# DCDmllm/AnyEdit

Measured on NVIDIA H100. Metric: edited images/sec (512x512, 50-step DDIM, CFG), higher is better.
Workload: dtype f16

## Files before the change

### anyedit_b200/_lib.py

```python
import ctypes as C
import os

_HERE = os.path.dirname(os.path.abspath(__file__))
LIB_PATH = os.path.join(_HERE, "libanysd_b200.so")

F32, F16, I64 = 0, 1, 2
EINVAL, ECUDA, EUNSUPPORTED = -1, -2, -3


class GemmParams(C.Structure):
    _fields_ = [
        ("A", C.c_void_p), ("W", C.c_void_p), ("bias", C.c_void_p), ("rowadd", C.c_void_p),
        ("residual", C.c_void_p), ("out", C.c_void_p),
        ("M", C.c_int), ("N", C.c_int), ("K", C.c_int),
        ("lda", C.c_int), ("ldw", C.c_int), ("ldo", C.c_int), ("ldr", C.c_int), ("ld_rowadd", C.c_int),
        ("rows_per_batch", C.c_int), ("act", C.c_int), ("out_dtype", C.c_int), ("conv", C.c_int),
        ("Nimg", C.c_int), ("H", C.c_int), ("Wd", C.c_int), ("Cin", C.c_int),
        ("stride", C.c_int), ("upsample", C.c_int),
        ("workspace", C.c_void_p), ("workspace_bytes", C.c_size_t),
        ("conv_pad", C.c_int),
        ("stats", C.c_void_p), ("stats_images", C.c_int),
        ("splitk_workspace", C.c_void_p), ("splitk_workspace_bytes", C.c_size_t),
        ("splitk_counters", C.c_void_p), ("splitk_counters_bytes", C.c_size_t),
        ("row_stats", C.c_void_p), ("ln_stats", C.c_void_p), ("ln_colsum", C.c_void_p), ("ln_eps", C.c_float),
# ... 48 lines not shown
    "anysd_add_nchw_into_nhwc_f16": (_I, [_VP, _I, _VP, _I, _I, _I, _I, _VP]),
    "anysd_nhwc_to_nchw": (_I, [_VP, _I, _I, _VP, _I, _I, _I, _I, _I, _VP]),
    "anysd_concat_channels_f16": (_I, [_VP, _I, _VP, _I, _VP, _LL, _VP]),
    "anysd_cast_f32_to_f16": (_I, [_VP, _VP, _LL, _VP]),
    "anysd_timestep_embedding_f16": (_I, [_VP, _I, _VP, _I, _I, _F, _VP]),
    "anysd_emb_finalize": (_I, [_VP, _VP, _VP, _I, _VP, _VP, _I, _I, _VP]),
    "anysd_router_gate_f32": (_I, [_VP, _VP, _I, _VP, _VP, _VP, _I, _I, _I, _I, _VP]),
    "anysd_groupnorm_workspace_bytes": (_SZ, [_I, _I, _I]),
    "anysd_groupnorm_resident": (_I, [_I, _I, _I, _I]),
    "anysd_groupnorm_nhwc_f16": (_I, [_VP, _I, _VP, _I, _VP, _VP, _VP, _I, _I, _I, _F, _I, _VP, _SZ, _VP]),
    "anysd_layernorm_f16": (_I, [_VP, _VP, _VP, _VP, _LL, _I, _F, _VP]),
    "anysd_gemm_f16": (_I, [C.POINTER(GemmParams), _VP]),
    "anysd_gemm_stats_slabs": (_I, [C.POINTER(GemmParams)]),
    "anysd_gemm_splitk_workspace_bytes": (_SZ, [C.POINTER(GemmParams)]),
    "anysd_geglu_ff_f16": (_I, [_VP, _I, _VP, _VP, _VP, _VP, _VP, _I, _VP, _I, _I, _I, _I, _VP]),
    "anysd_groupnorm_apply_nhwc_f16": (_I, [_VP, _I, _VP, _I, _VP, _I, _VP, _VP, _VP, _I, _I, _I, _F, _I, _VP, _SZ, _VP]),
    "anysd_attention_f16": (_I, [C.POINTER(AttnParams), _VP]),
    "anysd_cfg_ddim_step_f32": (_I, [_VP, _VP, _VP, _VP, _F, _I, _I, _VP, _VP, _LL, _I, _VP]),
    "anysd_cfg3_ddim_step_f32": (_I, [_VP, _VP, _VP, _VP, _F, _F, _VP, _VP, _LL, _I, _VP]),
    "anysd_cfg_plms_step_f32": (_I, [_VP, _VP, _VP, _F, _I, _VP, _VP, _VP, _LL, _I, _VP]),
    "anysd_cfg_dpmpp_step_f32": (_I, [_VP, _VP, _VP, _F, _I, _VP, _VP, _VP, _LL, _I, _VP]),
    "anysd_softmax_rows_f32": (_I, [_VP, _LL, _VP, _LL, _I, _I, _F, _VP]),
    "anysd_gaussian_posterior_f32": (_I, [_VP, _VP, _VP, _VP, _F, _I, _LL, _VP]),
    "anysd_embed_tokens_f16": (_I, [_VP, _VP, _VP, _VP, _I, _I, _I, _I, _VP]),
    "anysd_attention_small_f16": (_I, [_VP, _VP, _VP, _VP, _I, _I, _I, _I, _I, _I, _I, _I, _I, _F, _I, _VP]),
    "anysd_resize_bilinear_f16": (_I, [_VP, _VP, _VP, _I, _I, _I, _I, _I, _I, _I, _I, _VP]),
    "anysd_resize_bilinear_ac_f32": (_I, [_VP, _VP, _I, _I, _I, _I, _I, _VP]),
    "anysd_relu_f16": (_I, [_VP, _VP, _LL, _VP]),
    "anysd_depth_to_space_f16": (_I, [_VP, _VP, _I, _I, _I, _I, _I, _VP]),
    "anysd_space_to_depth_f16": (_I, [_VP, _VP, _I, _I, _I, _I, _I, _VP]),
# ... 67 lines not shown
```

### anyedit_b200/csrc/common.cuh

```cuda
#pragma once
#include <cuda_fp16.h>
#include <cuda_runtime.h>
#include <stdint.h>
#include <stdio.h>

#include "../../include/anysd_b200.h"

namespace anysd {

void set_error(const char* fmt, ...);
int check_launch(const char* what);

#define ANYSD_REQUIRE(cond, code, ...)                 \
    do {                                               \
        if (!(cond)) {                                 \
            ::anysd::set_error(__VA_ARGS__);           \
            return (code);                             \
        }                                              \
    } while (0)

static inline int cdiv(long long a, long long b) { return (int)((a + b - 1) / b); }

int sm_count();

// ... 35 lines not shown
#pragma unroll
    for (int i = 0; i < 4; ++i) {
        float2 t = __half22float2(h[i]);
        f[2 * i] = t.x;
        f[2 * i + 1] = t.y;
    }
}
__device__ __forceinline__ uint4 pack8(const float* f) {
    uint4 u;
    __half2* h = reinterpret_cast<__half2*>(&u);
#pragma unroll
    for (int i = 0; i < 4; ++i) h[i] = __floats2half2_rn(f[2 * i], f[2 * i + 1]);
    return u;
}

__device__ __forceinline__ uint32_t smem_u32(const void* p) {
    return (uint32_t)__cvta_generic_to_shared(p);
}

__device__ __forceinline__ void cp_async16(uint32_t dst, const void* src, bool valid) {
    int sz = valid ? 16 : 0;
    asm volatile("cp.async.cg.shared.global [%0], [%1], 16, %2;\n" ::"r"(dst), "l"(src), "r"(sz));
}
__device__ __forceinline__ void cp_async_commit() { asm volatile("cp.async.commit_group;\n" ::); }
template <int N>
__device__ __forceinline__ void cp_async_wait() {
    asm volatile("cp.async.wait_group %0;\n" ::"n"(N));
}

__device__ __forceinline__ void ldmatrix_x4(uint32_t& r0, uint32_t& r1, uint32_t& r2, uint32_t& r3, uint32_t addr) {
// ... 18 lines not shown
```

### anyedit_b200/csrc/norm.cu

```cuda
#include "common.cuh"

namespace anysd {

constexpr int GN_MAX_SPLITS = 64;
constexpr int GN_U = 8;

__device__ __forceinline__ float silu_fast(float v) {
    float e, r;
    asm("ex2.approx.ftz.f32 %0, %1;" : "=f"(e) : "f"(v * -1.4426950408889634f));
    asm("rcp.approx.ftz.f32 %0, %1;" : "=f"(r) : "f"(1.0f + e));
    return v * r;
}

struct GnGeom {
    int CV;
    int CV1;
    int R;
    int T;
};

static GnGeom gn_geom(int C1, int C2) {
    GnGeom g;
    g.CV = (C1 + C2) / 8;
    g.CV1 = C1 / 8;
// ... 471 lines not shown
template <int LPR, int VPL>
__global__ void layernorm_kernel(const uint4* __restrict__ x, const float* __restrict__ gamma,
                                 const float* __restrict__ beta, uint4* __restrict__ y, long long M, int CV, float eps) {
    constexpr int RPW = 32 / LPR;
    const int lane = threadIdx.x & 31;
    const int sub = lane / LPR, l = lane % LPR;
    const long long row = ((long long)blockIdx.x * (blockDim.x >> 5) + (threadIdx.x >> 5)) * RPW + sub;
    const bool row_ok = row < M;
    const uint4* xr = x + (row_ok ? row : 0) * CV;
    float f[VPL][8];
    float s = 0.f;
#pragma unroll
    for (int i = 0; i < VPL; ++i) {
        const int v = l + i * LPR;
        if (v < CV) {
            uint4 u = __ldg(xr + v);
            unpack8(u, f[i]);
#pragma unroll
            for (int j = 0; j < 8; ++j) s += f[i][j];
        }
    }
#pragma unroll
    for (int o = LPR / 2; o > 0; o >>= 1) s += __shfl_xor_sync(0xffffffffu, s, o);
    const float inv_c = 1.0f / (float)(CV * 8);
    const float mean = s * inv_c;
    float q = 0.f;
#pragma unroll
    for (int i = 0; i < VPL; ++i) {
        const int v = l + i * LPR;
        if (v < CV) {
#pragma unroll
            for (int j = 0; j < 8; ++j) {
                float d = f[i][j] - mean;
                q += d * d;
            }
        }
    }
#pragma unroll
    for (int o = LPR / 2; o > 0; o >>= 1) q += __shfl_xor_sync(0xffffffffu, q, o);
    const float rstd = rsqrtf(q * inv_c + eps);
    if (!row_ok) return;
    uint4* yr = y + row * CV;
#pragma unroll
    for (int i = 0; i < VPL; ++i) {
        const int v = l + i * LPR;
        if (v < CV) {
            const float4* g4 = reinterpret_cast<const float4*>(gamma + v * 8);
            const float4* b4 = reinterpret_cast<const float4*>(beta + v * 8);
            float4 g0 = __ldg(g4), g1 = __ldg(g4 + 1), b0 = __ldg(b4), b1 = __ldg(b4 + 1);
            float gg[8] = {g0.x, g0.y, g0.z, g0.w, g1.x, g1.y, g1.z, g1.w};
            float bb[8] = {b0.x, b0.y, b0.z, b0.w, b1.x, b1.y, b1.z, b1.w};
            float o[8];
#pragma unroll
            for (int j = 0; j < 8; ++j) o[j] = (f[i][j] - mean) * rstd * gg[j] + bb[j];
            yr[v] = pack8(o);
        }
    }
}

}

using namespace anysd;

extern "C" {

int anysd_groupnorm_resident(int C1, int C2, int HW, int G) {
    GnResPlan pl;
    return gn_res_plan(C1, C2 < 0 ? 0 : C2, HW, G, &pl) ? 1 : 0;
}

size_t anysd_groupnorm_workspace_bytes(int N, int G, int C) {
// ... 125 lines not shown
```

### anyedit_b200/csrc/wgmma.cuh

```cuda
#pragma once
#include <stdint.h>

namespace anysd {

__device__ __forceinline__ void wg_fence() { asm volatile("wgmma.fence.sync.aligned;" ::: "memory"); }
__device__ __forceinline__ void wg_commit() { asm volatile("wgmma.commit_group.sync.aligned;" ::: "memory"); }
template <int N>
__device__ __forceinline__ void wg_wait() { asm volatile("wgmma.wait_group.sync.aligned %0;" ::"n"(N) : "memory"); }
__device__ __forceinline__ void wg_fence_regs(float& r) { asm volatile("" : "+f"(r)::"memory"); }

__device__ __forceinline__ uint64_t wg_desc(uint32_t addr, uint32_t lbo_bytes, uint32_t sbo_bytes) {
    return (uint64_t)((addr >> 4) & 0x3FFF) | ((uint64_t)((lbo_bytes >> 4) & 0x3FFF) << 16) |
           ((uint64_t)((sbo_bytes >> 4) & 0x3FFF) << 32) | (1ull << 62);
}

template <int N>
struct Wgmma;

template <>
struct Wgmma<16> {
    static __device__ __forceinline__ void ss(float* d, uint64_t a, uint64_t b, int scale_d) {
        asm volatile(
            "{\n\t.reg .pred p;\n\tsetp.ne.b32 p, %10, 0;\n\t"
            "wgmma.mma_async.sync.aligned.m64n16k16.f32.f16.f16 {%0, %1, %2, %3, %4, %5, %6, %7}, %8, %9, p, 1, 1, 0, 0;\n\t}"
// ... 56 lines not shown
            "{\n\t.reg .pred p;\n\tsetp.ne.b32 p, %37, 0;\n\t"
            "wgmma.mma_async.sync.aligned.m64n64k16.f32.f16.f16 {%0, %1, %2, %3, %4, %5, %6, %7, %8, %9, %10, %11, %12, %13, %14, %15, %16, %17, %18, %19, %20, %21, %22, %23, %24, %25, %26, %27, %28, %29, %30, %31}, {%32, %33, %34, %35}, %36, p, 1, 1, 1;\n\t}"
            : "+f"(d[0]), "+f"(d[1]), "+f"(d[2]), "+f"(d[3]), "+f"(d[4]), "+f"(d[5]), "+f"(d[6]), "+f"(d[7]), "+f"(d[8]), "+f"(d[9]), "+f"(d[10]), "+f"(d[11]), "+f"(d[12]), "+f"(d[13]), "+f"(d[14]), "+f"(d[15]), "+f"(d[16]), "+f"(d[17]), "+f"(d[18]), "+f"(d[19]), "+f"(d[20]), "+f"(d[21]), "+f"(d[22]), "+f"(d[23]), "+f"(d[24]), "+f"(d[25]), "+f"(d[26]), "+f"(d[27]), "+f"(d[28]), "+f"(d[29]), "+f"(d[30]), "+f"(d[31])
            : "r"(a[0]), "r"(a[1]), "r"(a[2]), "r"(a[3]), "l"(b), "r"(scale_d));
    }
};
template <>
struct Wgmma<80> {
    static __device__ __forceinline__ void ss(float* d, uint64_t a, uint64_t b, int scale_d) {
        asm volatile(
            "{\n\t.reg .pred p;\n\tsetp.ne.b32 p, %42, 0;\n\t"
            "wgmma.mma_async.sync.aligned.m64n80k16.f32.f16.f16 {%0, %1, %2, %3, %4, %5, %6, %7, %8, %9, %10, %11, %12, %13, %14, %15, %16, %17, %18, %19, %20, %21, %22, %23, %24, %25, %26, %27, %28, %29, %30, %31, %32, %33, %34, %35, %36, %37, %38, %39}, %40, %41, p, 1, 1, 0, 0;\n\t}"
            : "+f"(d[0]), "+f"(d[1]), "+f"(d[2]), "+f"(d[3]), "+f"(d[4]), "+f"(d[5]), "+f"(d[6]), "+f"(d[7]), "+f"(d[8]), "+f"(d[9]), "+f"(d[10]), "+f"(d[11]), "+f"(d[12]), "+f"(d[13]), "+f"(d[14]), "+f"(d[15]), "+f"(d[16]), "+f"(d[17]), "+f"(d[18]), "+f"(d[19]), "+f"(d[20]), "+f"(d[21]), "+f"(d[22]), "+f"(d[23]), "+f"(d[24]), "+f"(d[25]), "+f"(d[26]), "+f"(d[27]), "+f"(d[28]), "+f"(d[29]), "+f"(d[30]), "+f"(d[31]), "+f"(d[32]), "+f"(d[33]), "+f"(d[34]), "+f"(d[35]), "+f"(d[36]), "+f"(d[37]), "+f"(d[38]), "+f"(d[39])
            : "l"(a), "l"(b), "r"(scale_d));
    }
    static __device__ __forceinline__ void rs_t(float* d, const uint32_t* a, uint64_t b, int scale_d) {
        asm volatile(
            "{\n\t.reg .pred p;\n\tsetp.ne.b32 p, %45, 0;\n\t"
            "wgmma.mma_async.sync.aligned.m64n80k16.f32.f16.f16 {%0, %1, %2, %3, %4, %5, %6, %7, %8, %9, %10, %11, %12, %13, %14, %15, %16, %17, %18, %19, %20, %21, %22, %23, %24, %25, %26, %27, %28, %29, %30, %31, %32, %33, %34, %35, %36, %37, %38, %39}, {%40, %41, %42, %43}, %44, p, 1, 1, 1;\n\t}"
            : "+f"(d[0]), "+f"(d[1]), "+f"(d[2]), "+f"(d[3]), "+f"(d[4]), "+f"(d[5]), "+f"(d[6]), "+f"(d[7]), "+f"(d[8]), "+f"(d[9]), "+f"(d[10]), "+f"(d[11]), "+f"(d[12]), "+f"(d[13]), "+f"(d[14]), "+f"(d[15]), "+f"(d[16]), "+f"(d[17]), "+f"(d[18]), "+f"(d[19]), "+f"(d[20]), "+f"(d[21]), "+f"(d[22]), "+f"(d[23]), "+f"(d[24]), "+f"(d[25]), "+f"(d[26]), "+f"(d[27]), "+f"(d[28]), "+f"(d[29]), "+f"(d[30]), "+f"(d[31]), "+f"(d[32]), "+f"(d[33]), "+f"(d[34]), "+f"(d[35]), "+f"(d[36]), "+f"(d[37]), "+f"(d[38]), "+f"(d[39])
            : "r"(a[0]), "r"(a[1]), "r"(a[2]), "r"(a[3]), "l"(b), "r"(scale_d));
    }
};
template <>
struct Wgmma<96> {
    static __device__ __forceinline__ void ss(float* d, uint64_t a, uint64_t b, int scale_d) {
        asm volatile(
            "{\n\t.reg .pred p;\n\tsetp.ne.b32 p, %50, 0;\n\t"
            "wgmma.mma_async.sync.aligned.m64n96k16.f32.f16.f16 {%0, %1, %2, %3, %4, %5, %6, %7, %8, %9, %10, %11, %12, %13, %14, %15, %16, %17, %18, %19, %20, %21, %22, %23, %24, %25, %26, %27, %28, %29, %30, %31, %32, %33, %34, %35, %36, %37, %38, %39, %40, %41, %42, %43, %44, %45, %46, %47}, %48, %49, p, 1, 1, 0, 0;\n\t}"
            : "+f"(d[0]), "+f"(d[1]), "+f"(d[2]), "+f"(d[3]), "+f"(d[4]), "+f"(d[5]), "+f"(d[6]), "+f"(d[7]), "+f"(d[8]), "+f"(d[9]), "+f"(d[10]), "+f"(d[11]), "+f"(d[12]), "+f"(d[13]), "+f"(d[14]), "+f"(d[15]), "+f"(d[16]), "+f"(d[17]), "+f"(d[18]), "+f"(d[19]), "+f"(d[20]), "+f"(d[21]), "+f"(d[22]), "+f"(d[23]), "+f"(d[24]), "+f"(d[25]), "+f"(d[26]), "+f"(d[27]), "+f"(d[28]), "+f"(d[29]), "+f"(d[30]), "+f"(d[31]), "+f"(d[32]), "+f"(d[33]), "+f"(d[34]), "+f"(d[35]), "+f"(d[36]), "+f"(d[37]), "+f"(d[38]), "+f"(d[39]), "+f"(d[40]), "+f"(d[41]), "+f"(d[42]), "+f"(d[43]), "+f"(d[44]), "+f"(d[45]), "+f"(d[46]), "+f"(d[47])
// ... 114 lines not shown
```

### anyedit_b200/ops.py

```python
import os
import ctypes as C

import torch

from . import _lib
from ._lib import F16, F32, I64, AttnParams, GemmParams

_DT = {torch.float32: F32, torch.float16: F16, torch.int64: I64}

launch_count = 0


def _stream():
    return C.c_void_p(torch.cuda.current_stream().cuda_stream)


def _ptr(t):
    return C.c_void_p(t.data_ptr()) if t is not None else None


def _cuda(*ts):
    for t in ts:
        if t is not None and not t.is_cuda:
            raise _lib.AnysdError("anysd_b200 ops need CUDA tensors; there is no CPU fallback")
# ... 236 lines not shown
    _cuda(x, w1, b1, w2t, b2, residual, out)
    Cc = x.shape[-1]
    M = x.numel() // Cc
    hidden = w2t.shape[0]
    assert w1.shape == (2 * hidden, Cc) and w2t.shape == (hidden, Cc) and b1.numel() == 2 * hidden
    assert b1.dtype == torch.float32 and b2.dtype == torch.float32 and b1.is_contiguous() and b2.is_contiguous()
    assert w1.is_contiguous() and w2t.is_contiguous()
    fl = 2.0 * M * (2 * hidden) * Cc + 2.0 * M * Cc * hidden
    with _Traced("gemm", fl, f"ff-geglu M={M} C={Cc} hidden={hidden}"):
        _lib.check(_lib.load().anysd_geglu_ff_f16(_ptr(x), x.stride(-2), _ptr(w1), _ptr(b1), _ptr(w2t), _ptr(b2),
                                                  _ptr(residual), residual.stride(-2), _ptr(out), out.stride(-2), M, Cc,
                                                  hidden, _stream()), "geglu_ff")
    _count()


def conv3x3(x, W, out, bias=None, rowadd=None, residual=None, stride=1, upsample=0, ld_rowadd=None,
            logical_cin=None, logical_cout=None, act=0, pad_rb=False, stats=False):
    _cuda(x, W, out)
    Nimg, H, Wd, Cin = x.shape
    Hl, Wl = H << upsample, Wd << upsample
    if pad_rb:
        assert stride == 2 and not upsample
        Ho, Wo = (Hl - 2) // 2 + 1, (Wl - 2) // 2 + 1
    else:
        Ho, Wo = (Hl - 1) // stride + 1, (Wl - 1) // stride + 1
    p = GemmParams()
    p.A, p.W, p.out = x.data_ptr(), W.data_ptr(), out.data_ptr()
    p.bias = bias.data_ptr() if bias is not None else None
    p.rowadd = rowadd.data_ptr() if rowadd is not None else None
    p.residual = residual.data_ptr() if residual is not None else None
# ... 477 lines not shown
```

### anyedit_b200/unet.py

```python
import math
import os

import torch
import torch.nn as nn

from . import ops



class _Param(nn.Module):

    def __init__(self, wshape, bias=True, kind="linear", zero=False):
        super().__init__()
        self.kind = kind
        self.weight = nn.Parameter(torch.empty(*wshape))
        if bias:
            self.bias = nn.Parameter(torch.empty(wshape[0]))
        else:
            self.register_parameter("bias", None)
        self.reset(zero)

    @torch.no_grad()
    def reset(self, zero=False):
        if self.kind == "norm":
# ... 99 lines not shown
        super().__init__()
        self.conv = _Param((out_ch, ch, 3, 3), kind="conv")


class _Embedding(nn.Module):
    def __init__(self, n, d):
        super().__init__()
        self.weight = nn.Parameter(torch.randn(n, d))



_LN_FOLD = os.environ.get("ANYSD_LN_FOLD", "0")[:1] == "1"


FF_FUSED_C = 320


def ff1_chunk_order(hidden, chunk=32):
    idx = []
    for c in range(hidden // chunk):
        for P in range(chunk):
            i, q = divmod(P, 4)
            u = c * chunk + 16 * (i // 4) + (2 * q, 2 * q + 1, 2 * q + 8, 2 * q + 9)[i % 4]
            idx += [2 * u, 2 * u + 1]
    return torch.tensor(idx, dtype=torch.long)


def _h(t, dev):
    return t.detach().to(device=dev, dtype=torch.float16).contiguous()

# ... 452 lines not shown
                ops.gemm(xq, ln[1]["w"], qkv, bias=ln[1]["b"], ln=(ln[0], ln[1]["cs"], 1e-5))
            else:
                ops.gemm(xq, ad["qkv_w"], qkv, bias=ad["qkv_b"])
            ops.attention(qkv, qkv[:, Cp:], qkv[:, 2 * Cp:], a, N, ad["heads"], n_q, n_q, ad["d"],
                          3 * Cp, 3 * Cp, 3 * Cp, C, head_stride=hs, aux_cols=ad["aux"])
        else:
            L = ctx.shape[1]
            if q_pre is not None:
                q = q_pre
            else:
                q = torch.empty(N * n_q, Cp, dtype=torch.float16, device=dev)
                if ln is not None:
                    ops.gemm(xq, ln[1]["w"], q, bias=ln[1]["b"], ln=(ln[0], ln[1]["cs"], 1e-5))
                else:
                    ops.gemm(xq, ad["q_w"], q)
            kvc, xl = st.get("kvc"), st.get("xl", 0)
            if kvc is not None and kvc["mode"] == "use":
                kv = kvc["bufs"][xl]
            else:
                have = kvc is not None and len(kvc["bufs"]) > xl
                kv = kvc["bufs"][xl] if have else torch.empty(N * L, 2 * Cp, dtype=torch.float16, device=dev)
                ops.gemm(ctx.view(N * L, -1), ad["kv_w"], kv, bias=ad["kv_b"])
                if kvc is not None and not have:
                    kvc["bufs"].append(kv)
            st["xl"] = xl + 1
            ops.attention(q, kv, kv[:, Cp:], a, N, ad["heads"], n_q, L, ad["d"], Cp, 2 * Cp, 2 * Cp, C, head_stride=hs,
                          aux_cols=ad["aux"])
            if expert and st["anysd"] is not None and st["anysd"].get("experts") is not None:
                st["anysd"]["experts"](st["layer"], q, a, N, n_q, ad["heads"], ad["d"], hs, ad["aux"])
            if expert:
                st["layer"] += 1
        if out_stats:
            out._ln = ops.row_stats_buffer(N * n_q, C, dev)
        ops.gemm(a, ad["o_w"], out, bias=ad["o_b"], residual=residual, row_stats=out._ln if out_stats else None)

    @staticmethod
    def _ln_folded(b):
        fb = b.get("_fold")
        if fb is None:
            def fold(w16, bias, gamma, beta):
                w32 = w16.float()
                wf = (w32 * gamma[None, :]).to(torch.float16).contiguous()
                bb = w32 @ beta
                if bias is not None:
                    bb = bb + bias
                return {"w": wf, "cs": wf.float().sum(1).contiguous(), "b": bb.contiguous()}
            a1 = b["attn1"]
            fb = {"a1": fold(a1["qkv_w"], a1["qkv_b"], b["ln1_w"], b["ln1_b"]) if b["self"] else fold(a1["q_w"], None, b["ln1_w"], b["ln1_b"]),
                  "a2": fold(b["attn2"]["q_w"], None, b["ln2_w"], b["ln2_b"]),
# ... 22 lines not shown
        inner = d["inner"]
        dev = h.device
        g = torch.empty_like(h)
        ops.groupnorm(h, d["gn_w"], d["gn_b"], g, N, n, 1e-6, False, st["ws"], stats=getattr(h, "_gn", None))
        t = torch.empty(M, inner, dtype=torch.float16, device=dev)
        fold0 = _LN_FOLD and inner % 64 == 0
        if fold0:
            t._ln = ops.row_stats_buffer(M, inner, dev)
        ops.gemm(g.view(M, C), d["pin_w"], t, bias=d["pin_b"], row_stats=t._ln if fold0 else None)
        for i, b in enumerate(d["blocks"]):
            ctx = st["ctx"][i] if i < len(st["ctx"]) else st["ctx"][-1]
            if share and not b["self"]:
                t, h = self._dup_rows(t), self._dup_rows(h)
                N, M, share = 2 * N, 2 * M, False
            fold = _LN_FOLD and inner % 64 == 0
            if fold:
                fb = self._ln_folded(b)
                t2 = torch.empty_like(t)
                self._attn(b["attn1"], t, None if b["self"] else ctx, N, n, st, b["self"], t, t2, ln=(t._ln, fb["a1"]), out_stats=True)
            else:
                ln = torch.empty_like(t)
                ops.layernorm(t, b["ln1_w"], b["ln1_b"], ln)
                t2 = torch.empty_like(t)
                if b["self"]:
                    self._attn(b["attn1"], ln, None, N, n, st, True, t, t2)
                else:
                    self._attn(b["attn1"], ln, ctx, N, n, st, False, t, t2)
                ln2 = torch.empty_like(t)
                ops.layernorm(t2, b["ln2_w"], b["ln2_b"], ln2)
            if ctx is None:
# ... 38 lines not shown
```

### include/anysd_b200.h

```cpp
#ifndef ANYSD_B200_H_
#define ANYSD_B200_H_

#include <stddef.h>
#include <stdint.h>

#ifdef __cplusplus
extern "C" {
#endif

#define ANYSD_OK 0
#define ANYSD_EINVAL (-1)
#define ANYSD_ECUDA (-2)
#define ANYSD_EUNSUPPORTED (-3)

#define ANYSD_F32 0
#define ANYSD_F16 1
#define ANYSD_I64 2

typedef void* anysd_stream_t;

const char* anysd_last_error(void);
int anysd_version(void);
int anysd_device_info(int* sm_count, int* cc_major, int* cc_minor);

// ... 50 lines not shown
    void* splitk_workspace;
    size_t splitk_workspace_bytes;
    void* splitk_counters;
    size_t splitk_counters_bytes;
    float* row_stats;
    const float* ln_stats;
    const float* ln_colsum;
    float ln_eps;
    const float* col_scale;
} anysd_gemm_params;
int anysd_gemm_f16(const anysd_gemm_params* p, anysd_stream_t stream);
int anysd_gemm_stats_slabs(const anysd_gemm_params* p);
size_t anysd_gemm_splitk_workspace_bytes(const anysd_gemm_params* p);
int anysd_geglu_ff_f16(const void* x, int ldx, const void* w1, const float* b1, const void* w2t, const float* b2,
                       const void* residual, int ldr, void* out, int ldo, int M, int C, int hidden, anysd_stream_t stream);

typedef struct {
    const void* q; const void* k; const void* v; void* out;
    long long q_batch_stride, k_batch_stride, v_batch_stride, o_batch_stride;
    int ld_q, ld_k, ld_v, ld_o;
    int B, heads, n_q, n_kv, d;
    float scale;
    const float* gate;
    int gate_stride;
    int accumulate;
    int head_stride;
    int aux_cols;
    float* lse;
} anysd_attn_params;
int anysd_attention_f16(const anysd_attn_params* p, anysd_stream_t stream);
// ... 128 lines not shown
```

Measured before the change: 4.233.

## Fuse attn1 out-proj, LN2, cross-attention and LN3 into one wgmma kernel

Adds a warp-specialized Hopper kernel for the C=320 transformer blocks. One producer warp streams weights and context K/V through a TMA/mbarrier double-buffered ring. Two consumer warpgroups run, per tile, the attn1 output projection plus residual, LayerNorm2, per-head Q projection, cross-attention over up to 80 keys, the attn2 output projection plus residual, and LayerNorm3, keeping intermediates in shared memory and registers. This removes several kernel launches and global-memory round trips of the activations. The trade-offs are very high register pressure (160 accumulator floats per thread) and one CTA per SM. The path is taken only when LN folding is off and the block shape matches (8 heads, d=40, n a multiple of 128, no experts).

Measured after the change: 4.369 (median of 6 runs). 3.2% higher.

```diff
diff --git a/anyedit_b200/_lib.py b/anyedit_b200/_lib.py
--- a/anyedit_b200/_lib.py
+++ b/anyedit_b200/_lib.py
@@ -86,6 +86,7 @@
     "anysd_gemm_stats_slabs": (_I, [C.POINTER(GemmParams)]),
     "anysd_gemm_splitk_workspace_bytes": (_SZ, [C.POINTER(GemmParams)]),
     "anysd_geglu_ff_f16": (_I, [_VP, _I, _VP, _VP, _VP, _VP, _VP, _I, _VP, _I, _I, _I, _I, _VP]),
+    "anysd_xattn_block_f16": (_I, [_VP] * 8 + [_I] + [_VP] * 7 + [_I] * 8 + [_F, _VP]),
     "anysd_groupnorm_apply_nhwc_f16": (_I, [_VP, _I, _VP, _I, _VP, _I, _VP, _VP, _VP, _I, _I, _I, _F, _I, _VP, _SZ, _VP]),
     "anysd_attention_f16": (_I, [C.POINTER(AttnParams), _VP]),
     "anysd_cfg_ddim_step_f32": (_I, [_VP, _VP, _VP, _VP, _F, _I, _I, _VP, _VP, _LL, _I, _VP]),
diff --git a/anyedit_b200/csrc/common.cuh b/anyedit_b200/csrc/common.cuh
--- a/anyedit_b200/csrc/common.cuh
+++ b/anyedit_b200/csrc/common.cuh
@@ -73,6 +73,45 @@
     return u;
 }
 
+template <int LPR, int VPL>
+__device__ __forceinline__ void layernorm_row_stats(const float (&f)[VPL][8], float s, int l, int CV, float eps,
+                                                    float& mean, float& rstd) {
+#pragma unroll
+    for (int o = LPR / 2; o > 0; o >>= 1) s += __shfl_xor_sync(0xffffffffu, s, o);
+    const float inv_c = 1.0f / (float)(CV * 8);
+    mean = __fmul_rn(s, inv_c);
+    float q = 0.f;
+#pragma unroll
+    for (int i = 0; i < VPL; ++i)
+        if (l + i * LPR < CV) {
+#pragma unroll
+            for (int j = 0; j < 8; ++j) {
+                float d = f[i][j] - mean;
+                q += d * d;
+            }
+        }
+#pragma unroll
+    for (int o = LPR / 2; o > 0; o >>= 1) q += __shfl_xor_sync(0xffffffffu, q, o);
+    rstd = rsqrtf(q * inv_c + eps);
+}
+template <int LPR, int VPL>
+__device__ __forceinline__ void layernorm_row_apply(float (&f)[VPL][8], int l, int CV, const float* __restrict__ gamma,
+                                                    const float* __restrict__ beta, float mean, float rstd) {
+#pragma unroll
+    for (int i = 0; i < VPL; ++i) {
+        const int v = l + i * LPR;
+        if (v < CV) {
+            const float4* g4 = reinterpret_cast<const float4*>(gamma + v * 8);
+            const float4* b4 = reinterpret_cast<const float4*>(beta + v * 8);
+            float4 g0 = __ldg(g4), g1 = __ldg(g4 + 1), b0 = __ldg(b4), b1 = __ldg(b4 + 1);
+            float gg[8] = {g0.x, g0.y, g0.z, g0.w, g1.x, g1.y, g1.z, g1.w};
+            float bb[8] = {b0.x, b0.y, b0.z, b0.w, b1.x, b1.y, b1.z, b1.w};
+#pragma unroll
+            for (int j = 0; j < 8; ++j) f[i][j] = (f[i][j] - mean) * rstd * gg[j] + bb[j];
+        }
+    }
+}
+
 __device__ __forceinline__ uint32_t smem_u32(const void* p) {
     return (uint32_t)__cvta_generic_to_shared(p);
 }
diff --git a/anyedit_b200/csrc/norm.cu b/anyedit_b200/csrc/norm.cu
--- a/anyedit_b200/csrc/norm.cu
+++ b/anyedit_b200/csrc/norm.cu
@@ -509,47 +509,20 @@
     for (int i = 0; i < VPL; ++i) {
         const int v = l + i * LPR;
         if (v < CV) {
-            uint4 u = __ldg(xr + v);
-            unpack8(u, f[i]);
+            unpack8(__ldg(xr + v), f[i]);
 #pragma unroll
             for (int j = 0; j < 8; ++j) s += f[i][j];
         }
     }
-#pragma unroll
-    for (int o = LPR / 2; o > 0; o >>= 1) s += __shfl_xor_sync(0xffffffffu, s, o);
-    const float inv_c = 1.0f / (float)(CV * 8);
-    const float mean = s * inv_c;
-    float q = 0.f;
+    float mean, rstd;
+    layernorm_row_stats<LPR, VPL>(f, s, l, CV, eps, mean, rstd);
+    if (!row_ok) return;
+    layernorm_row_apply<LPR, VPL>(f, l, CV, gamma, beta, mean, rstd);
+    uint4* yr = y + row * CV;
 #pragma unroll
     for (int i = 0; i < VPL; ++i) {
         const int v = l + i * LPR;
-        if (v < CV) {
-#pragma unroll
-            for (int j = 0; j < 8; ++j) {
-                float d = f[i][j] - mean;
-                q += d * d;
-            }
-        }
-    }
-#pragma unroll
-    for (int o = LPR / 2; o > 0; o >>= 1) q += __shfl_xor_sync(0xffffffffu, q, o);
-    const float rstd = rsqrtf(q * inv_c + eps);
-    if (!row_ok) return;
-    uint4* yr = y + row * CV;
-#pragma unroll
-    for (int i = 0; i < VPL; ++i) {
-        const int v = l + i * LPR;
-        if (v < CV) {
-            const float4* g4 = reinterpret_cast<const float4*>(gamma + v * 8);
-            const float4* b4 = reinterpret_cast<const float4*>(beta + v * 8);
-            float4 g0 = __ldg(g4), g1 = __ldg(g4 + 1), b0 = __ldg(b4), b1 = __ldg(b4 + 1);
-            float gg[8] = {g0.x, g0.y, g0.z, g0.w, g1.x, g1.y, g1.z, g1.w};
-            float bb[8] = {b0.x, b0.y, b0.z, b0.w, b1.x, b1.y, b1.z, b1.w};
-            float o[8];
-#pragma unroll
-            for (int j = 0; j < 8; ++j) o[j] = (f[i][j] - mean) * rstd * gg[j] + bb[j];
-            yr[v] = pack8(o);
-        }
+        if (v < CV) yr[v] = pack8(f[i]);
     }
 }
 
diff --git a/anyedit_b200/csrc/wgmma.cuh b/anyedit_b200/csrc/wgmma.cuh
--- a/anyedit_b200/csrc/wgmma.cuh
+++ b/anyedit_b200/csrc/wgmma.cuh
@@ -94,6 +94,13 @@
             : "+f"(d[0]), "+f"(d[1]), "+f"(d[2]), "+f"(d[3]), "+f"(d[4]), "+f"(d[5]), "+f"(d[6]), "+f"(d[7]), "+f"(d[8]), "+f"(d[9]), "+f"(d[10]), "+f"(d[11]), "+f"(d[12]), "+f"(d[13]), "+f"(d[14]), "+f"(d[15]), "+f"(d[16]), "+f"(d[17]), "+f"(d[18]), "+f"(d[19]), "+f"(d[20]), "+f"(d[21]), "+f"(d[22]), "+f"(d[23]), "+f"(d[24]), "+f"(d[25]), "+f"(d[26]), "+f"(d[27]), "+f"(d[28]), "+f"(d[29]), "+f"(d[30]), "+f"(d[31]), "+f"(d[32]), "+f"(d[33]), "+f"(d[34]), "+f"(d[35]), "+f"(d[36]), "+f"(d[37]), "+f"(d[38]), "+f"(d[39])
             : "l"(a), "l"(b), "r"(scale_d));
     }
+    static __device__ __forceinline__ void rs(float* d, const uint32_t* a, uint64_t b, int scale_d) {
+        asm volatile(
+            "{\n\t.reg .pred p;\n\tsetp.ne.b32 p, %45, 0;\n\t"
+            "wgmma.mma_async.sync.aligned.m64n80k16.f32.f16.f16 {%0, %1, %2, %3, %4, %5, %6, %7, %8, %9, %10, %11, %12, %13, %14, %15, %16, %17, %18, %19, %20, %21, %22, %23, %24, %25, %26, %27, %28, %29, %30, %31, %32, %33, %34, %35, %36, %37, %38, %39}, {%40, %41, %42, %43}, %44, p, 1, 1, 0;\n\t}"
+            : "+f"(d[0]), "+f"(d[1]), "+f"(d[2]), "+f"(d[3]), "+f"(d[4]), "+f"(d[5]), "+f"(d[6]), "+f"(d[7]), "+f"(d[8]), "+f"(d[9]), "+f"(d[10]), "+f"(d[11]), "+f"(d[12]), "+f"(d[13]), "+f"(d[14]), "+f"(d[15]), "+f"(d[16]), "+f"(d[17]), "+f"(d[18]), "+f"(d[19]), "+f"(d[20]), "+f"(d[21]), "+f"(d[22]), "+f"(d[23]), "+f"(d[24]), "+f"(d[25]), "+f"(d[26]), "+f"(d[27]), "+f"(d[28]), "+f"(d[29]), "+f"(d[30]), "+f"(d[31]), "+f"(d[32]), "+f"(d[33]), "+f"(d[34]), "+f"(d[35]), "+f"(d[36]), "+f"(d[37]), "+f"(d[38]), "+f"(d[39])
+            : "r"(a[0]), "r"(a[1]), "r"(a[2]), "r"(a[3]), "l"(b), "r"(scale_d));
+    }
     static __device__ __forceinline__ void rs_t(float* d, const uint32_t* a, uint64_t b, int scale_d) {
         asm volatile(
             "{\n\t.reg .pred p;\n\tsetp.ne.b32 p, %45, 0;\n\t"
diff --git a/anyedit_b200/csrc/xattn_block_wgmma.cu b/anyedit_b200/csrc/xattn_block_wgmma.cu
--- /dev/null
+++ b/anyedit_b200/csrc/xattn_block_wgmma.cu
@@ -0,0 +1,428 @@
+#include <cuda.h>
+
+#include "common.cuh"
+#include "wgmma.cuh"
+
+namespace anysd {
+
+constexpr int XB_C = 320, XB_BM = 128, XB_THREADS = 384;
+constexpr int XB_HEADS = 8, XB_D = 40, XB_HS = 48, XB_KEYS = 80;
+constexpr int XB_KA = XB_C / 64;
+constexpr int XB_X_ATOM = XB_BM * 128;
+constexpr int XB_X_BYTES = XB_KA * XB_X_ATOM;
+constexpr int XB_WA = 192, XB_WB = XB_C - XB_WA;
+constexpr int XB_WQ_ATOM = XB_HS * 128;
+constexpr int XB_KV_ATOM = XB_KEYS * 128;
+constexpr int XB_SLOT = XB_KA * XB_WQ_ATOM;
+static_assert(XB_WA * 128 <= XB_SLOT && 2 * XB_KV_ATOM <= XB_SLOT, "cross-attention block: ring slot");
+constexpr int XB_A2_OFF = XB_X_BYTES;
+constexpr int XB_RING_OFF = XB_A2_OFF + XB_X_BYTES;
+constexpr int XB_BAR_OFF = XB_RING_OFF + 2 * XB_SLOT;
+constexpr int XB_SMEM = XB_BAR_OFF + 8 * 8 + 1024;
+static_assert(XB_SMEM <= 227 * 1024, "cross-attention block: shared memory");
+
+struct XbArgs {
+    const __half* t;
+    const float *bo1, *ln2_w, *ln2_b, *bo2, *ln3_w, *ln3_b;
+    __half *t2, *t3, *l3;
+    int n, L, num_tiles;
+    float eps;
+};
+
+__device__ __forceinline__ void xb_init(uint32_t bar, uint32_t count) {
+    asm volatile("mbarrier.init.shared::cta.b64 [%0], %1;" ::"r"(bar), "r"(count));
+}
+__device__ __forceinline__ void xb_expect_tx(uint32_t bar, uint32_t bytes) {
+    asm volatile("mbarrier.arrive.expect_tx.shared::cta.b64 _, [%0], %1;" ::"r"(bar), "r"(bytes) : "memory");
+}
+__device__ __forceinline__ void xb_arrive(uint32_t bar) {
+    asm volatile("mbarrier.arrive.shared::cta.b64 _, [%0];" ::"r"(bar) : "memory");
+}
+__device__ __forceinline__ void xb_wait(uint32_t bar, uint32_t parity) {
+    asm volatile(
+        "{\n\t"
+        ".reg .pred P1;\n\t"
+        "WAIT_LOOP:\n\t"
+        "mbarrier.try_wait.parity.shared::cta.b64 P1, [%0], %1;\n\t"
+        "@P1 bra DONE;\n\t"
+        "bra WAIT_LOOP;\n\t"
+        "DONE:\n\t"
+        "}" ::"r"(bar), "r"(parity) : "memory");
+}
+__device__ __forceinline__ void xb_tma_2d(uint32_t dst, const CUtensorMap* tm, uint32_t bar, int c0, int c1) {
+    asm volatile("cp.async.bulk.tensor.2d.shared::cluster.global.mbarrier::complete_tx::bytes [%0], [%1, {%3, %4}], [%2];"
+                 ::"r"(dst), "l"(tm), "r"(bar), "r"(c0), "r"(c1) : "memory");
+}
+__device__ __forceinline__ float xb_ex2(float x) {
+    float y;
+    asm("ex2.approx.ftz.f32 %0, %1;" : "=f"(y) : "f"(x));
+    return y;
+}
+__device__ __forceinline__ uint32_t xb_pack(float a, float b) {
+    __half2 h = __floats2half2_rn(a, b);
+    return *reinterpret_cast<uint32_t*>(&h);
+}
+__device__ __forceinline__ void xb_fence_async() { asm volatile("fence.proxy.async.shared::cta;" ::: "memory"); }
+__device__ __forceinline__ void xb_wg_sync(int wg) { asm volatile("bar.sync %0, 128;" ::"r"(1 + wg) : "memory"); }
+__device__ __forceinline__ uint32_t xb_swz(int row, int col, int atom_bytes) {
+    return (col >> 6) * atom_bytes + row * 128 + ((((col >> 3) & 7) ^ (row & 7)) << 4) + (col & 7) * 2;
+}
+
+__global__ void __launch_bounds__(XB_THREADS, 1)
+xattn_block_wgmma_kernel(const __grid_constant__ CUtensorMap tmX, const __grid_constant__ CUtensorMap tmWo1a,
+                         const __grid_constant__ CUtensorMap tmWo1b, const __grid_constant__ CUtensorMap tmWq,
+                         const __grid_constant__ CUtensorMap tmKV, const __grid_constant__ CUtensorMap tmWo2a,
+                         const __grid_constant__ CUtensorMap tmWo2b, const XbArgs p) {
+    extern __shared__ unsigned char xb_smem_raw[];
+    const uint32_t raw = smem_u32(xb_smem_raw);
+    const uint32_t base = (raw + 1023u) & ~1023u;
+    unsigned char* smem = xb_smem_raw + (base - raw);
+    const uint32_t bars = base + XB_BAR_OFF;
+    auto BAR = [&](int i) { return bars + 8u * i; };
+    auto slot = [&](uint32_t c) { return base + XB_RING_OFF + (c & 1) * XB_SLOT; };
+    const int warp = threadIdx.x >> 5, lane = threadIdx.x & 31;
+
+    if (threadIdx.x == 0) {
+        asm volatile("prefetch.tensormap [%0];" ::"l"(&tmX) : "memory");
+        asm volatile("prefetch.tensormap [%0];" ::"l"(&tmWo1a) : "memory");
+        asm volatile("prefetch.tensormap [%0];" ::"l"(&tmWo1b) : "memory");
+        asm volatile("prefetch.tensormap [%0];" ::"l"(&tmWq) : "memory");
+        asm volatile("prefetch.tensormap [%0];" ::"l"(&tmKV) : "memory");
+        asm volatile("prefetch.tensormap [%0];" ::"l"(&tmWo2a) : "memory");
+        asm volatile("prefetch.tensormap [%0];" ::"l"(&tmWo2b) : "memory");
+        for (int i = 0; i < 6; ++i) xb_init(BAR(i), (i == 1 || i >= 4) ? 8 : 1);
+        asm volatile("fence.mbarrier_init.release.cluster;" ::: "memory");
+    }
+    __syncthreads();
+
+    if (warp < 4) {
+        asm volatile("setmaxnreg.dec.sync.aligned.u32 24;" ::: "memory");
+        if (warp == 0 && lane == 0) {
+            uint32_t c = 0;
+            auto push = [&](uint32_t bytes) {
+                const int s = c & 1;
+                xb_wait(BAR(4 + s), ((c >> 1) & 1) ^ 1);
+                xb_expect_tx(BAR(2 + s), bytes);
+                return slot(c++);
+            };
+            auto push_wo = [&](const CUtensorMap* ta, const CUtensorMap* tb) {
+                for (int kb = 0; kb < XB_KA; ++kb) {
+                    uint32_t d = push(XB_WA * 128);
+                    xb_tma_2d(d, ta, BAR(2 + ((c - 1) & 1)), kb * 64, 0);
+                    d = push(XB_WB * 128);
+                    xb_tma_2d(d, tb, BAR(2 + ((c - 1) & 1)), kb * 64, XB_WA);
+                }
+            };
+            int it = 0;
+            for (int tile = blockIdx.x; tile < p.num_tiles; tile += gridDim.x, ++it) {
+                const int img = tile * XB_BM / p.n;
+                xb_wait(BAR(1), (it & 1) ^ 1);
+                xb_expect_tx(BAR(0), XB_X_BYTES);
+                for (int a = 0; a < XB_KA; ++a) xb_tma_2d(base + a * XB_X_ATOM, &tmX, BAR(0), a * 64, tile * XB_BM);
+                push_wo(&tmWo1a, &tmWo1b);
+                for (int h = 0; h < XB_HEADS; ++h) {
+                    uint32_t d = push(XB_SLOT);
+                    for (int a = 0; a < XB_KA; ++a) xb_tma_2d(d + a * XB_WQ_ATOM, &tmWq, BAR(2 + ((c - 1) & 1)), a * 64, h * XB_HS);
+                    d = push(2 * XB_KV_ATOM);
+                    xb_tma_2d(d, &tmKV, BAR(2 + ((c - 1) & 1)), h * XB_HS, img * p.L);
+                    xb_tma_2d(d + XB_KV_ATOM, &tmKV, BAR(2 + ((c - 1) & 1)), XB_HEADS * XB_HS + h * XB_HS, img * p.L);
+                }
+                push_wo(&tmWo2a, &tmWo2b);
+            }
+        }
+        return;
+    }
+
+    asm volatile("setmaxnreg.inc.sync.aligned.u32 240;" ::: "memory");
+    const int wg = __shfl_sync(0xffffffffu, (warp >> 2) - 1, 0);
+    const int wq = warp & 3, q4 = lane & 3, wtid = threadIdx.x - 128 * (wg + 1);
+    const uint32_t xa = base + wg * 64 * 128, a2a = base + XB_A2_OFF + wg * 64 * 128;
+    unsigned char* xs_g = smem + wg * 64 * 128;
+    unsigned char* a2_g = smem + XB_A2_OFF + wg * 64 * 128;
+    float o[XB_C / 2];
+    uint32_t c = 0;
+
+    auto take = [&]() { xb_wait(BAR(2 + (c & 1)), (c >> 1) & 1); };
+    auto give = [&](uint32_t cc) {
+        __syncwarp();
+        if (lane == 0) xb_arrive(BAR(4 + (cc & 1)));
+    };
+    auto product_wo = [&](uint32_t a_base) {
+#pragma unroll
+        for (int i = 0; i < XB_C / 2; ++i) o[i] = 0.f;
+        wg_fence();
+#pragma unroll 1
+        for (int kb = 0; kb < XB_KA; ++kb) {
+            take();
+#pragma unroll
+            for (int k = 0; k < 4; ++k)
+                Wgmma<XB_WA>::ss(o, wg_desc(a_base + kb * XB_X_ATOM + k * 32, 16, 1024), wg_desc(slot(c) + k * 32, 16, 1024), 1);
+            wg_commit();
+            if (kb > 0) {
+                wg_wait<1>();
+                give(c - 1);
+            }
+            ++c;
+            take();
+#pragma unroll
+            for (int k = 0; k < 4; ++k)
+                Wgmma<XB_WB>::ss(o + XB_WA / 2, wg_desc(a_base + kb * XB_X_ATOM + k * 32, 16, 1024),
+                                 wg_desc(slot(c) + k * 32, 16, 1024), 1);
+            wg_commit();
+            wg_wait<1>();
+            give(c - 1);
+            ++c;
+        }
+        wg_wait<0>();
+        give(c - 1);
+#pragma unroll
+        for (int i = 0; i < XB_C / 2; ++i) wg_fence_regs(o[i]);
+    };
+    auto epilogue_wo = [&](int tile, const float* bias, const __half* res, __half* dst) {
+#pragma unroll
+        for (int h = 0; h < 2; ++h) {
+            const int rr = wq * 16 + (lane >> 2) + 8 * h;
+            const size_t m = (size_t)tile * XB_BM + wg * 64 + rr;
+            const __half* rrow = res + m * XB_C + 2 * q4;
+            __half* orow = dst + m * XB_C + 2 * q4;
+            constexpr int G = 8;
+#pragma unroll
+            for (int i0 = 0; i0 < XB_C / 8; i0 += G) {
+                __half2 rv[G];
+#pragma unroll
+                for (int u = 0; u < G; ++u) rv[u] = *reinterpret_cast<const __half2*>(rrow + 8 * (i0 + u));
+#pragma unroll
+                for (int u = 0; u < G; ++u) {
+                    const int i = i0 + u;
+                    const float2 bb = __ldg(reinterpret_cast<const float2*>(bias + 8 * i + 2 * q4));
+                    float v0 = o[4 * i + 2 * h] + bb.x, v1 = o[4 * i + 2 * h + 1] + bb.y;
+                    v0 += 0.f;
+                    v1 += 0.f;
+                    const float2 r = __half22float2(rv[u]);
+                    v0 += r.x;
+                    v1 += r.y;
+                    const __half2 hv = __floats2half2_rn(v0, v1);
+                    *reinterpret_cast<__half2*>(orow + 8 * i) = hv;
+                    *reinterpret_cast<__half2*>(xs_g + xb_swz(rr, 8 * i + 2 * q4, XB_X_ATOM)) = hv;
+                }
+            }
+        }
+    };
+    auto layernorm = [&](int tile, const float* gamma, const float* beta, __half* out) {
+        const int l = wtid & 7;
+#pragma unroll 1
+        for (int pass = 0; pass < 4; ++pass) {
+            const int rr = pass * 16 + (wtid >> 3);
+            float f[5][8];
+            float s = 0.f;
+#pragma unroll
+            for (int i = 0; i < 5; ++i) {
+                unpack8(*reinterpret_cast<const uint4*>(xs_g + xb_swz(rr, 8 * (l + 8 * i), XB_X_ATOM)), f[i]);
+#pragma unroll
+                for (int j = 0; j < 8; ++j) s += f[i][j];
+            }
+            float mean, rstd;
+            layernorm_row_stats<8, 5>(f, s, l, XB_C / 8, p.eps, mean, rstd);
+            layernorm_row_apply<8, 5>(f, l, XB_C / 8, gamma, beta, mean, rstd);
+#pragma unroll
+            for (int i = 0; i < 5; ++i) {
+                const uint4 u = pack8(f[i]);
+                if (out != nullptr)
+                    *reinterpret_cast<uint4*>(out + ((size_t)tile * XB_BM + wg * 64 + rr) * XB_C + 8 * (l + 8 * i)) = u;
+                else
+                    *reinterpret_cast<uint4*>(xs_g + xb_swz(rr, 8 * (l + 8 * i), XB_X_ATOM)) = u;
+            }
+        }
+    };
+
+    int it = 0;
+    for (int tile = blockIdx.x; tile < p.num_tiles; tile += gridDim.x, ++it) {
+        xb_wait(BAR(0), it & 1);
+        product_wo(xa);
+        epilogue_wo(tile, p.bo1, p.t, p.t2);
+        xb_wg_sync(wg);
+        layernorm(tile, p.ln2_w, p.ln2_b, nullptr);
+        xb_fence_async();
+        xb_wg_sync(wg);
+
+#pragma unroll 1
+        for (int hh = 0; hh < XB_HEADS; ++hh) {
+            float qc[XB_HS / 2];
+#pragma unroll
+            for (int i = 0; i < XB_HS / 2; ++i) qc[i] = 0.f;
+            take();
+            wg_fence();
+#pragma unroll
+            for (int k = 0; k < XB_C / 16; ++k)
+                Wgmma<XB_HS>::ss(qc, wg_desc(xa + (k >> 2) * XB_X_ATOM + (k & 3) * 32, 16, 1024),
+                                 wg_desc(slot(c) + (k >> 2) * XB_WQ_ATOM + (k & 3) * 32, 16, 1024), 1);
+            wg_commit();
+            wg_wait<0>();
+            give(c);
+            ++c;
+            uint32_t qa[XB_HS / 16][4];
+#pragma unroll
+            for (int i = 0; i < XB_HS / 2; ++i) {
+                wg_fence_regs(qc[i]);
+                qc[i] += 0.f;
+            }
+#pragma unroll
+            for (int s = 0; s < XB_HS / 16; ++s) {
+                const float* t = qc + 8 * s;
+                qa[s][0] = xb_pack(t[0], t[1]);
+                qa[s][1] = xb_pack(t[2], t[3]);
+                qa[s][2] = xb_pack(t[4], t[5]);
+                qa[s][3] = xb_pack(t[6], t[7]);
+            }
+            take();
+            const uint32_t kb = slot(c), vb = kb + XB_KV_ATOM;
+            float sc[XB_KEYS / 2];
+            wg_fence();
+#pragma unroll
+            for (int k = 0; k < XB_HS / 16; ++k) Wgmma<XB_KEYS>::rs(sc, qa[k], wg_desc(kb + k * 32, 16, 1024), k > 0);
+            wg_commit();
+            wg_wait<0>();
+#pragma unroll
+            for (int i = 0; i < XB_KEYS / 2; ++i) wg_fence_regs(sc[i]);
+#pragma unroll
+            for (int i = 0; i < XB_KEYS / 8; ++i)
+#pragma unroll
+                for (int e = 0; e < 4; ++e)
+                    if (8 * i + 2 * q4 + (e & 1) >= p.L) sc[4 * i + e] = -INFINITY;
+            float mx[2] = {-INFINITY, -INFINITY}, lr[2] = {0.f, 0.f};
+#pragma unroll
+            for (int i = 0; i < XB_KEYS / 8; ++i)
+#pragma unroll
+                for (int e = 0; e < 4; ++e) mx[e >> 1] = fmaxf(mx[e >> 1], sc[4 * i + e]);
+#pragma unroll
+            for (int r = 0; r < 2; ++r) {
+                mx[r] = fmaxf(mx[r], __shfl_xor_sync(0xffffffffu, mx[r], 1));
+                mx[r] = fmaxf(mx[r], __shfl_xor_sync(0xffffffffu, mx[r], 2));
+            }
+            uint32_t pa[XB_KEYS / 16][4];
+#pragma unroll
+            for (int kk = 0; kk < XB_KEYS / 16; ++kk) {
+                float* t = sc + 8 * kk;
+#pragma unroll
+                for (int e = 0; e < 8; ++e) t[e] = xb_ex2(t[e] - mx[(e >> 1) & 1]);
+                lr[0] += (t[0] + t[1]) + (t[4] + t[5]);
+                lr[1] += (t[2] + t[3]) + (t[6] + t[7]);
+                pa[kk][0] = xb_pack(t[0], t[1]);
+                pa[kk][1] = xb_pack(t[2], t[3]);
+                pa[kk][2] = xb_pack(t[4], t[5]);
+                pa[kk][3] = xb_pack(t[6], t[7]);
+            }
+            float oh[XB_HS / 2];
+#pragma unroll
+            for (int i = 0; i < XB_HS / 2; ++i) oh[i] = 0.f;
+            wg_fence();
+#pragma unroll
+            for (int kk = 0; kk < XB_KEYS / 16; ++kk)
+                Wgmma<XB_HS>::rs_t(oh, pa[kk], wg_desc(vb + kk * 2048, XB_KV_ATOM, 1024), 1);
+            wg_commit();
+            wg_wait<0>();
+#pragma unroll
+            for (int i = 0; i < XB_HS / 2; ++i) wg_fence_regs(oh[i]);
+            give(c);
+            ++c;
+#pragma unroll
+            for (int r = 0; r < 2; ++r) {
+                float l = lr[r];
+                l += __shfl_xor_sync(0xffffffffu, l, 1);
+                l += __shfl_xor_sync(0xffffffffu, l, 2);
+                const float inv = 1.0f / l;
+                const int rr = wq * 16 + (lane >> 2) + 8 * r;
+#pragma unroll
+                for (int i = 0; i < XB_D / 8; ++i)
+                    *reinterpret_cast<__half2*>(a2_g + xb_swz(rr, hh * XB_D + 8 * i + 2 * q4, XB_X_ATOM)) =
+                        __floats2half2_rn(oh[4 * i + 2 * r] * inv, oh[4 * i + 2 * r + 1] * inv);
+            }
+        }
+        xb_fence_async();
+        xb_wg_sync(wg);
+
+        product_wo(a2a);
+        epilogue_wo(tile, p.bo2, p.t2, p.t3);
+        xb_wg_sync(wg);
+        layernorm(tile, p.ln3_w, p.ln3_b, p.l3);
+        xb_fence_async();
+        __syncwarp();
+        if (lane == 0) xb_arrive(BAR(1));
+    }
+}
+
+typedef CUresult (*EncodeTiledFnX)(CUtensorMap*, CUtensorMapDataType, cuuint32_t, void*, const cuuint64_t*,
+                                   const cuuint64_t*, const cuuint32_t*, const cuuint32_t*, CUtensorMapInterleave,
+                                   CUtensorMapSwizzle, CUtensorMapL2promotion, CUtensorMapFloatOOBfill);
+static EncodeTiledFnX x_get_encode() {
+    static EncodeTiledFnX fn = nullptr;
+    static bool tried = false;
+    if (!tried) {
+        tried = true;
+        void* f = nullptr;
+        cudaDriverEntryPointQueryResult qr;
+        if (cudaGetDriverEntryPoint("cuTensorMapEncodeTiled", &f, cudaEnableDefault, &qr) == cudaSuccess &&
+            qr == cudaDriverEntryPointSuccess)
+            fn = (EncodeTiledFnX)f;
+    }
+    return fn;
+}
+static bool x_map(CUtensorMap* tm, const void* ptr, uint64_t width, uint64_t rows, uint64_t ld, uint32_t box_rows) {
+    cuuint64_t dims[2] = {width, rows};
+    cuuint64_t strides[1] = {ld * 2};
+    cuuint32_t box[2] = {64, box_rows};
+    cuuint32_t es[2] = {1, 1};
+    return x_get_encode()(tm, CU_TENSOR_MAP_DATA_TYPE_FLOAT16, 2, const_cast<void*>(ptr), dims, strides, box, es,
+                          CU_TENSOR_MAP_INTERLEAVE_NONE, CU_TENSOR_MAP_SWIZZLE_128B, CU_TENSOR_MAP_L2_PROMOTION_L2_256B,
+                          CU_TENSOR_MAP_FLOAT_OOB_FILL_NONE) == CUDA_SUCCESS;
+}
+
+}
+
+using namespace anysd;
+
+extern "C" int anysd_xattn_block_f16(const void* a1, const void* t, const void* wo1, const float* bo1, const float* ln2_w,
+                                     const float* ln2_b, const void* wq, const void* kv, int ld_kv, const void* wo2,
+                                     const float* bo2, const float* ln3_w, const float* ln3_b, void* t2, void* t3, void* l3,
+                                     int M, int n, int L, int C, int heads, int d, int hs, int aux_cols, float eps,
+                                     anysd_stream_t stream) {
+    ANYSD_REQUIRE(a1 && t && wo1 && bo1 && ln2_w && ln2_b && wq && kv && wo2 && bo2 && ln3_w && ln3_b && t2 && t3 && l3,
+                  ANYSD_EINVAL, "xattn_block: null pointer");
+    ANYSD_REQUIRE(M > 0 && n > 0 && L > 0 && M % n == 0, ANYSD_EINVAL, "xattn_block: bad M=%d n=%d L=%d", M, n, L);
+    ANYSD_REQUIRE(C == XB_C && heads == XB_HEADS && d == XB_D && hs == XB_HS, ANYSD_EUNSUPPORTED,
+                  "xattn_block: only C = %d as %d heads of %d (stride %d) (got C=%d heads=%d d=%d hs=%d)", XB_C, XB_HEADS,
+                  XB_D, XB_HS, C, heads, d, hs);
+    ANYSD_REQUIRE(aux_cols, ANYSD_EUNSUPPORTED, "xattn_block: only aux_cols heads");
+    ANYSD_REQUIRE(n % XB_BM == 0, ANYSD_EUNSUPPORTED, "xattn_block: rows per image n=%d must be a multiple of %d", n, XB_BM);
+    ANYSD_REQUIRE(L <= XB_KEYS, ANYSD_EUNSUPPORTED, "xattn_block: context of %d tokens (at most %d)", L, XB_KEYS);
+    ANYSD_REQUIRE(ld_kv >= 2 * heads * hs && ld_kv % 8 == 0, ANYSD_EINVAL, "xattn_block: ld_kv=%d", ld_kv);
+    const void* ptrs[] = {a1, t, wo1, bo1, ln2_w, ln2_b, wq, kv, wo2, bo2, ln3_w, ln3_b, t2, t3, l3};
+    for (const void* q : ptrs) ANYSD_REQUIRE(((uintptr_t)q % 16) == 0, ANYSD_EINVAL, "xattn_block: pointers must be 16-byte aligned");
+    ANYSD_REQUIRE(x_get_encode() != nullptr, ANYSD_ECUDA, "xattn_block: cuTensorMapEncodeTiled unavailable");
+    const int B = M / n;
+    CUtensorMap tmX, tmWo1a, tmWo1b, tmWq, tmKV, tmWo2a, tmWo2b;
+    const bool ok = x_map(&tmX, a1, XB_C, (uint64_t)M, XB_C, XB_BM) && x_map(&tmWo1a, wo1, XB_C, XB_C, XB_C, XB_WA) &&
+                    x_map(&tmWo1b, wo1, XB_C, XB_C, XB_C, XB_WB) && x_map(&tmWq, wq, XB_C, XB_HEADS * XB_HS, XB_C, XB_HS) &&
+                    x_map(&tmKV, kv, 2 * XB_HEADS * XB_HS, (uint64_t)B * L, ld_kv, XB_KEYS) &&
+                    x_map(&tmWo2a, wo2, XB_C, XB_C, XB_C, XB_WA) && x_map(&tmWo2b, wo2, XB_C, XB_C, XB_C, XB_WB);
+    ANYSD_REQUIRE(ok, ANYSD_ECUDA, "xattn_block: cuTensorMapEncodeTiled failed (M=%d L=%d)", M, L);
+    static bool done[64];
+    int dev = 0;
+    cudaGetDevice(&dev);
+    dev &= 63;
+    if (!done[dev]) {
+        cudaError_t e = cudaFuncSetAttribute(xattn_block_wgmma_kernel, cudaFuncAttributeMaxDynamicSharedMemorySize, XB_SMEM);
+        ANYSD_REQUIRE(e == cudaSuccess, ANYSD_ECUDA, "xattn_block: smem opt-in failed: %s", cudaGetErrorString(e));
+        done[dev] = true;
+    }
+    XbArgs a;
+    a.t = (const __half*)t;
+    a.bo1 = bo1; a.ln2_w = ln2_w; a.ln2_b = ln2_b; a.bo2 = bo2; a.ln3_w = ln3_w; a.ln3_b = ln3_b;
+    a.t2 = (__half*)t2; a.t3 = (__half*)t3; a.l3 = (__half*)l3;
+    a.n = n; a.L = L; a.num_tiles = M / XB_BM; a.eps = eps;
+    int grid = sm_count();
+    if (grid > a.num_tiles) grid = a.num_tiles;
+    xattn_block_wgmma_kernel<<<grid, XB_THREADS, XB_SMEM, (cudaStream_t)stream>>>(tmX, tmWo1a, tmWo1b, tmWq, tmKV, tmWo2a,
+                                                                                  tmWo2b, a);
+    return check_launch("xattn_block (wgmma)");
+}
diff --git a/anyedit_b200/ops.py b/anyedit_b200/ops.py
--- a/anyedit_b200/ops.py
+++ b/anyedit_b200/ops.py
@@ -274,6 +274,23 @@
     _count()
 
 
+def xattn_block(a1, t, wo1, bo1, ln2_w, ln2_b, wq, kv, L, wo2, bo2, ln3_w, ln3_b, t2, t3, l3, n, heads, d, hs,
+                aux_cols=True, eps=1e-5):
+    _cuda(a1, t, wo1, bo1, ln2_w, ln2_b, wq, kv, wo2, bo2, ln3_w, ln3_b, t2, t3, l3)
+    Cc = a1.shape[-1]
+    M = a1.numel() // Cc
+    for x in (a1, t, t2, t3, l3, wo1, wo2, wq, bo1, bo2, ln2_w, ln2_b, ln3_w, ln3_b):
+        assert x.is_contiguous()
+    assert kv.stride(-1) == 1
+    B = M // n
+    fl = 2.0 * M * Cc * Cc * 2 + 2.0 * M * heads * d * Cc + 4.0 * B * heads * n * L * d
+    with _Traced("gemm", fl, f"xattn-block M={M} C={Cc} L={L}"):
+        _lib.check(_lib.load().anysd_xattn_block_f16(
+            _ptr(a1), _ptr(t), _ptr(wo1), _ptr(bo1), _ptr(ln2_w), _ptr(ln2_b), _ptr(wq), _ptr(kv), kv.stride(-2), _ptr(wo2),
+            _ptr(bo2), _ptr(ln3_w), _ptr(ln3_b), _ptr(t2), _ptr(t3), _ptr(l3), M, n, L, Cc, heads, d, hs, int(aux_cols),
+            float(eps), _stream()), "xattn_block")
+    _count()
+
 def conv3x3(x, W, out, bias=None, rowadd=None, residual=None, stride=1, upsample=0, ld_rowadd=None,
             logical_cin=None, logical_cout=None, act=0, pad_rb=False, stats=False):
     _cuda(x, W, out)
diff --git a/anyedit_b200/unet.py b/anyedit_b200/unet.py
--- a/anyedit_b200/unet.py
+++ b/anyedit_b200/unet.py
@@ -137,6 +137,7 @@
 
 
 FF_FUSED_C = 320
+XATTN_MAX_CTX = 80
 
 
 def ff1_chunk_order(hidden, chunk=32):
@@ -619,25 +620,40 @@
                     ops.gemm(xq, ln[1]["w"], q, bias=ln[1]["b"], ln=(ln[0], ln[1]["cs"], 1e-5))
                 else:
                     ops.gemm(xq, ad["q_w"], q)
-            kvc, xl = st.get("kvc"), st.get("xl", 0)
-            if kvc is not None and kvc["mode"] == "use":
-                kv = kvc["bufs"][xl]
-            else:
-                have = kvc is not None and len(kvc["bufs"]) > xl
-                kv = kvc["bufs"][xl] if have else torch.empty(N * L, 2 * Cp, dtype=torch.float16, device=dev)
-                ops.gemm(ctx.view(N * L, -1), ad["kv_w"], kv, bias=ad["kv_b"])
-                if kvc is not None and not have:
-                    kvc["bufs"].append(kv)
-            st["xl"] = xl + 1
+            kv = self._context_kv(ad, ctx, N, st)
             ops.attention(q, kv, kv[:, Cp:], a, N, ad["heads"], n_q, L, ad["d"], Cp, 2 * Cp, 2 * Cp, C, head_stride=hs,
                           aux_cols=ad["aux"])
             if expert and st["anysd"] is not None and st["anysd"].get("experts") is not None:
                 st["anysd"]["experts"](st["layer"], q, a, N, n_q, ad["heads"], ad["d"], hs, ad["aux"])
             if expert:
                 st["layer"] += 1
+        if out is None:
+            return a
         if out_stats:
             out._ln = ops.row_stats_buffer(N * n_q, C, dev)
         ops.gemm(a, ad["o_w"], out, bias=ad["o_b"], residual=residual, row_stats=out._ln if out_stats else None)
+
+    @staticmethod
+    def _context_kv(ad, ctx, N, st):
+        L, Cp = ctx.shape[1], ad["heads"] * ad["hs"]
+        kvc, xl = st.get("kvc"), st.get("xl", 0)
+        if kvc is not None and kvc["mode"] == "use":
+            kv = kvc["bufs"][xl]
+        else:
+            have = kvc is not None and len(kvc["bufs"]) > xl
+            kv = kvc["bufs"][xl] if have else torch.empty(N * L, 2 * Cp, dtype=torch.float16, device=ctx.device)
+            ops.gemm(ctx.view(N * L, -1), ad["kv_w"], kv, bias=ad["kv_b"])
+            if kvc is not None and not have:
+                kvc["bufs"].append(kv)
+        st["xl"] = xl + 1
+        return kv
+
+    @staticmethod
+    def _xattn_fused(b, ctx, n, st):
+        a2 = b["attn2"]
+        experts = st["anysd"] is not None and st["anysd"].get("experts") is not None
+        return ("ff1p_w" in b and b["self"] and not experts and ctx is not None and ctx.shape[1] <= XATTN_MAX_CTX
+                and n % 128 == 0 and a2["aux"] and (a2["heads"], a2["d"], a2["hs"]) == (8, 40, 48))
 
     @staticmethod
     def _ln_folded(b):
@@ -690,6 +706,23 @@
                 t, h = self._dup_rows(t), self._dup_rows(h)
                 N, M, share = 2 * N, 2 * M, False
             fold = _LN_FOLD and inner % 64 == 0
+            if not fold and self._xattn_fused(b, ctx, n, st):
+                ln = torch.empty_like(t)
+                ops.layernorm(t, b["ln1_w"], b["ln1_b"], ln)
+                a1 = self._attn(b["attn1"], ln, None, N, n, st, True, t, None)
+                if share:
+                    a1, t, h = self._dup_rows(a1), self._dup_rows(t), self._dup_rows(h)
+                    N, M, share = 2 * N, 2 * M, False
+                a1d, ad = b["attn1"], b["attn2"]
+                kv = self._context_kv(ad, ctx, N, st)
+                st["layer"] += 1
+                t2, t3, ln3 = (torch.empty_like(t) for _ in range(3))
+                ops.xattn_block(a1, t, a1d["o_w"], a1d["o_b"], b["ln2_w"], b["ln2_b"], ad["q_w"], kv, ctx.shape[1],
+                                ad["o_w"], ad["o_b"], b["ln3_w"], b["ln3_b"], t2, t3, ln3, n, ad["heads"], ad["d"], ad["hs"],
+                                aux_cols=ad["aux"])
+                t = torch.empty_like(t3)
+                ops.geglu_ff(ln3, b["ff1p_w"], b["ff1p_b"], b["ff2t_w"], b["ff2_b"], t3, t)
+                continue
             if fold:
                 fb = self._ln_folded(b)
                 t2 = torch.empty_like(t)
diff --git a/include/anysd_b200.h b/include/anysd_b200.h
--- a/include/anysd_b200.h
+++ b/include/anysd_b200.h
@@ -88,6 +88,10 @@
 size_t anysd_gemm_splitk_workspace_bytes(const anysd_gemm_params* p);
 int anysd_geglu_ff_f16(const void* x, int ldx, const void* w1, const float* b1, const void* w2t, const float* b2,
                        const void* residual, int ldr, void* out, int ldo, int M, int C, int hidden, anysd_stream_t stream);
+int anysd_xattn_block_f16(const void* a1, const void* t, const void* wo1, const float* bo1, const float* ln2_w,
+                          const float* ln2_b, const void* wq, const void* kv, int ld_kv, const void* wo2, const float* bo2,
+                          const float* ln3_w, const float* ln3_b, void* t2, void* t3, void* l3, int M, int n, int L, int C,
+                          int heads, int d, int hs, int aux_cols, float eps, anysd_stream_t stream);
 
 typedef struct {
     const void* q; const void* k; const void* v; void* out;
```
